# peterbudai/redux

Hardware: AMD Instinct MI355X
Metric: encode MB/s (whole node), per-block bitstream bit-exact (higher is better)
Workload: dtype u32

## Files before the change

redux_amd/csrc/redux_encode.hpp:

```cpp
#pragma once

#include "redux_coder.hpp"

#include "../../include/redux_hip.h"

#include <hip/hip_runtime.h>
#include <stdint.h>

namespace redux {

__global__ void k_fill_rc(double *rc, uint32_t n)
{
    const uint32_t i = blockIdx.x * blockDim.x + threadIdx.x;
    if (i < n) {
        const double r = 1.0 / (double)(257u + i);
        rc[i] = __longlong_as_double(__double_as_longlong(r) + 4);
    }
}

struct EncCore {
    const uint8_t *in;
    uint64_t       in_len;
    uint64_t       nblocks;
    uint8_t       *slots;
    uint64_t       slot_bytes;
    uint32_t      *sizes;
    int32_t       *status;
};

struct EncArgs : EncCore {
    const double  *rc;
    uint32_t       block_size;
    uint32_t       slot_cap;
    uint32_t       nfreeze;
    uint32_t       code_bits;
    uint32_t       aligned16;
    uint32_t       lanes;
    uint32_t      *claims;
    const redux_block *table;
    uint32_t       pair_width;
    uint32_t       win0, winlen;
    double         rc_frozen;
    uint32_t      *cstate, *cbase;
};
static_assert(sizeof(EncCore) == 56 && sizeof(EncArgs) == 144, "kernarg layout");

constexpr uint32_t kIdleEntry = 0xFFFFFFFFu;

struct EncLane {
    uint32_t soff, len;
    uint64_t ob;
};
__device__ __forceinline__ EncLane enc_lane(const EncArgs &a, uint64_t blk0, uint64_t blk, uint32_t lane, bool live, const uint8_t *&wsrc)
{
    EncLane L;
    if (a.table) {
        const redux_block e = a.table[live ? blk : blk0];
        wsrc   = a.in;
        L.soff = (uint32_t)e.offset;
        L.len  = live ? e.length : 0u;
        L.ob   = e.index;
    } else {
        wsrc   = a.in + blk0 * a.block_size;
        L.soff = live ? lane * a.block_size : 0u;
        L.len  = 0;
        if (live) {
            const uint64_t rem = a.in_len - blk * a.block_size;
            L.len              = rem < a.block_size ? (uint32_t)rem : a.block_size;
        }
        L.ob = blk;
    }
    return L;
}

__device__ __forceinline__ uint32_t wave_min(uint32_t v)
{
#pragma unroll
    for (int o = 32; o > 0; o >>= 1) {
        const uint32_t w = __shfl_xor(v, o);
        v = w < v ? w : v;
    }
    return v;
}
__device__ __forceinline__ uint32_t wave_max(uint32_t v)
{
#pragma unroll
    for (int o = 32; o > 0; o >>= 1) {
        const uint32_t w = __shfl_xor(v, o);
        v = w > v ? w : v;
    }
    return v;
}

template <bool U16, bool FIXUP, bool UPD>
__device__ __forceinline__ void encode_chunk(const Tree<U16> &T, EncState &S, const uint4 cur, uint32_t p,
                                             uint32_t nfreeze, rc_ptr rc, uint32_t sh, uint8_t *wdst)
{
    const uint32_t w[4] = {cur.x, cur.y, cur.z, cur.w};
    double         r[16];
#pragma unroll
    for (int i = 0; i < 16; i++)
        r[i] = rc[UPD ? p + i : nfreeze];
#pragma unroll
    for (int i = 0; i < 16; i++) {
        const uint32_t s   = (w[i >> 2] >> (8 * (i & 3))) & 0xFFu;
        const uint32_t nup = UPD ? p + i : nfreeze;
        uint32_t       lo, hi;
        T.template get_frequency<UPD>(s, nup, true, lo, hi);
        encode_symbol_fast<FIXUP>(S, lo, hi, 257u + nup, r[i], sh, wdst);
    }
}

template <bool U16, bool FIXUP>
__global__ void __launch_bounds__(64) k_encode(EncArgs a)
{
    __shared__ uint32_t lds[Tree<U16>::kDwords];
    const uint32_t lane = threadIdx.x;
    const uint64_t blk0 = (uint64_t)blockIdx.x * a.lanes;
    const uint64_t blk  = blk0 + lane;
    const bool     live = lane < a.lanes && blk < a.nblocks && !(a.table && a.table[blk].index == kIdleEntry);

    for (uint32_t i = lane; i < Tree<U16>::kDwords / 4; i += 64)
        reinterpret_cast<uint4 *>(lds)[i] = make_uint4(0, 0, 0, 0);
    __syncthreads();
    Tree<U16> T;
    T.init(lds, lane);

    const uint8_t *wsrc;
    const EncLane  EL    = enc_lane(a, blk0, blk, lane, live, wsrc);
    const uint32_t len   = EL.len, soff = EL.soff;
    uint8_t       *wdst  = a.slots + blk0 * a.slot_bytes;
    const uint32_t off0  = live ? lane * (uint32_t)a.slot_bytes
                                : (a.lanes == 1 ? 0u : (uint32_t)(a.nblocks - blk0) * (uint32_t)a.slot_bytes);
    const uint32_t limit = off0 + a.slot_cap;

    const uint32_t minlen  = __builtin_amdgcn_readfirstlane(wave_min(live ? len : 0xFFFFFFFFu));
    constexpr uint32_t kChunkBudget = 16 * 4 + 32;
    const uint32_t maxlen  = __builtin_amdgcn_readfirstlane(wave_max(live ? len : 0u));
    const uint32_t sh      = 32 - a.code_bits;
    const uint32_t nfreeze = a.nfreeze;
    const rc_ptr   rc      = (rc_ptr)a.rc;

    EncState S;
    enc_init(S, off0);

    uint32_t p        = 0;
    uint32_t main_end = 0;
    if (a.aligned16 && minlen != 0xFFFFFFFFu && minlen > 16)
        main_end = (minlen - 1) & ~15u;

    if (main_end) {
        const uint32_t a_end = main_end < (nfreeze & ~15u) ? main_end : (nfreeze & ~15u);
        if (p < a_end) {
            uint4 cur = *reinterpret_cast<const uint4 *>(wsrc + soff);
            for (; p < a_end; p += 16) {
                if (__builtin_amdgcn_ballot_w64(S.off + kChunkBudget > limit)) {
                    main_end = p;
                    break;
                }
                uint4 nxt = cur;
                if (p + 16 < a_end)
                    nxt = *reinterpret_cast<const uint4 *>(wsrc + soff + p + 16);
                encode_chunk<U16, FIXUP, true>(T, S, cur, p, nfreeze, rc, sh, wdst);
                cur = nxt;
            }
        }
        if (p < main_end && p < nfreeze) {
            const uint32_t m_end = p + 16;
            for (; p < m_end; p++) {
                const uint32_t nup = p < nfreeze ? p : nfreeze;
                uint32_t       lo, hi;
                T.template get_frequency<true>(wsrc[soff + p], nup, p < nfreeze, lo, hi);
                encode_symbol<FIXUP>(S, lo, hi, 257u + nup, rc[nup], sh, false, wdst, limit);
            }
        }
        if (p < main_end) {
            uint4 cur = *reinterpret_cast<const uint4 *>(wsrc + soff + p);
            for (; p < main_end; p += 16) {
                if (__builtin_amdgcn_ballot_w64(S.off + kChunkBudget > limit)) {
                    main_end = p;
                    break;
                }
                uint4 nxt = cur;
                if (p + 16 < main_end)
                    nxt = *reinterpret_cast<const uint4 *>(wsrc + soff + p + 16);
                encode_chunk<U16, FIXUP, false>(T, S, cur, p, nfreeze, rc, sh, wdst);
                cur = nxt;
            }
        }
    }

    for (; p <= maxlen; p++) {
        const uint32_t nup = p < nfreeze ? p : nfreeze;
        const double   r   = rc[nup];
        const uint32_t c   = 257u + nup;
        if (live && p < len) {
            uint32_t lo, hi;
            T.template get_frequency<true>(wsrc[soff + p], nup, p < nfreeze && p + 1 != len, lo, hi);
            encode_symbol<FIXUP>(S, lo, hi, c, r, sh, false, wdst, limit);
        } else if (live && p == len) {
            const uint32_t shifts = encode_symbol<FIXUP>(S, c - 1, c, c, r, sh, true, wdst, limit);
            const uint32_t size   = encode_finish(S, shifts, a.code_bits, off0, wdst, limit);
            a.sizes[EL.ob]  = size;
            a.status[EL.ob] = size > a.slot_cap ? REDUX_OUTPUT_TOO_SMALL : REDUX_OK;
        }
    }
}

constexpr uint32_t kRingSlots = 8;
constexpr uint32_t kRingBytes = 2 * kRingSlots * 64 * 8;

__device__ __forceinline__ void pair_barrier()
{
    asm volatile("s_waitcnt lgkmcnt(0)\n\ts_barrier" ::: "memory");
}

struct ChunkQueue {
    const uint8_t *base;
    uint32_t       soff;
    uint32_t       last;
    uint32_t       nextp;
    uint32_t       idx;
    uint4          c[8], n[8];

    __device__ __forceinline__ void prefetch()
    {
#pragma unroll
        for (int i = 0; i < 8; i++) {
            const uint32_t p = nextp + 16 * i;
            n[i] = *reinterpret_cast<const uint4 *>(base + soff + (p < last ? p : last));
        }
        nextp += 128;
    }
    __device__ __forceinline__ void swap()
    {
#pragma unroll
        for (int i = 0; i < 8; i++)
            c[i] = n[i];
        idx = 0;
        prefetch();
    }
    __device__ __forceinline__ void init(const uint8_t *b, uint32_t so, uint32_t e)
    {
        base = b; soff = so; last = e - 16; nextp = 0;
        prefetch();
        swap();
    }
    __device__ __forceinline__ uint4 pop()
    {
        uint4 r;
        switch (idx) {
        case 0: r = c[0]; break;
        case 1: r = c[1]; break;
        case 2: r = c[2]; break;
        case 3: r = c[3]; break;
        case 4: r = c[4]; break;
        case 5: r = c[5]; break;
        case 6: r = c[6]; break;
        default: r = c[7]; break;
        }
        if (++idx == 8)
            swap();
        return r;
    }
};

constexpr int kPairStride = 256 | kSwapped;
__device__ __forceinline__ uint32_t ring_at(uint32_t i, uint32_t lane)
{
    return (i >> 1) * 128u + lane * 2u + (i & 1u);
}
constexpr int kMaskAhead = 8;
static_assert(kMaskAhead == 4 || kMaskAhead == 8, "prime() covers these");
static_assert(16 % kMaskAhead == 0, "slot i % AHEAD must mean the same in every chunk");
struct MaskPipe {
    uint4    s[kMaskAhead], m[kMaskAhead];
    uint32_t four;
    __amdgpu_buffer_rsrc_t rsrc;
    __device__ __forceinline__ void init()
    {
        rsrc = __builtin_amdgcn_make_buffer_rsrc(const_cast<uint32_t *>(k_mask_table.v), 0, sizeof k_mask_table.v, 0x00027000);
        four = 4;
        asm volatile("" : "+v"(four));
    }
    __device__ __forceinline__ uint32_t row_of(int K, uint32_t w) const
    {
        uint32_t off;
        if (K == 0)
            asm("v_lshlrev_b32_sdwa %0, %1, %2 dst_sel:DWORD dst_unused:UNUSED_PAD src0_sel:DWORD src1_sel:BYTE_0" : "=v"(off) : "v"(four), "v"(w));
        else if (K == 1)
            asm("v_lshlrev_b32_sdwa %0, %1, %2 dst_sel:DWORD dst_unused:UNUSED_PAD src0_sel:DWORD src1_sel:BYTE_1" : "=v"(off) : "v"(four), "v"(w));
        else if (K == 2)
            asm("v_lshlrev_b32_sdwa %0, %1, %2 dst_sel:DWORD dst_unused:UNUSED_PAD src0_sel:DWORD src1_sel:BYTE_2" : "=v"(off) : "v"(four), "v"(w));
        else
            asm("v_lshlrev_b32_sdwa %0, %1, %2 dst_sel:DWORD dst_unused:UNUSED_PAD src0_sel:DWORD src1_sel:BYTE_3" : "=v"(off) : "v"(four), "v"(w));
        return off;
    }
    __device__ __forceinline__ void load(int slot, uint32_t row)
    {
        const char *e = reinterpret_cast<const char *>(k_mask_table.v) + row;
        (void)e;
        const auto r0 = __builtin_amdgcn_raw_buffer_load_b128(rsrc, row, 0, 0), r1 = __builtin_amdgcn_raw_buffer_load_b128(rsrc, row + 16u, 0, 0);
        s[slot] = make_uint4(r0[0], r0[1], r0[2], r0[3]);
        m[slot] = make_uint4(r1[0], r1[1], r1[2], r1[3]);
        const uint32_t sym = row >> 4;
    }
    __device__ __forceinline__ void prime(const uint4 cur)
    {
        init();
        const uint32_t w[2] = {cur.x, cur.y};
        load(0, row_of(0, w[0])); load(1, row_of(1, w[0])); load(2, row_of(2, w[0])); load(3, row_of(3, w[0]));
        if (kMaskAhead == 8) {
            load(4 % kMaskAhead, row_of(0, w[1])); load(5 % kMaskAhead, row_of(1, w[1]));
            load(6 % kMaskAhead, row_of(2, w[1])); load(7 % kMaskAhead, row_of(3, w[1]));
        }
    }
};

template <bool UPD>
__device__ __forceinline__ void model_chunk(const Tree<true> &T, uint2 *ring, uint32_t lane, const uint4 cur, const uint4 nxt,
                                            MaskPipe &mp, uint32_t p, uint32_t nfreeze, uint32_t *top = nullptr)
{
    constexpr int kInFlight = UPD ? 7 : 8;
    const uint32_t w[8] = {cur.x, cur.y, cur.z, cur.w, nxt.x, nxt.y, nxt.z, nxt.w};
    auto sym = [&](int i) { return (w[i >> 2] >> (8 * (i & 3))) & 0xFFu; };
    constexpr int D = 1;
    Tree<true>::Nodes q[D + 1];
    uint2             held = make_uint2(0, 0);
    constexpr bool kMasked = UPD && D == 1;
#pragma unroll
    for (int d = 0; d < D; d++)
        q[d] = kMasked ? T.issue_masked(sym(d), mp.s[d % kMaskAhead], top) : T.template issue<UPD>(sym(d), true, top);
#pragma unroll
    for (int i = 0; i < 16; i++) {
        const uint32_t s   = sym(i);
        const uint32_t nup = UPD ? p + i : nfreeze;
        const bool late = i == 7;
        if (i + D < 16 && !late) {
            q[D] = kMasked ? T.issue_masked(sym(i + D), mp.s[(i + D) % kMaskAhead], top) : T.template issue<UPD>(sym(i + D), true, top);
            __builtin_amdgcn_sched_barrier(0);
        }
        uint32_t lo, hi;
        if (D == 1 && i + D < 16 && !late && i != 8 && i != 0 && kInFlight == 7)
        {
            if (i & 1)
                __builtin_amdgcn_s_waitcnt(0xC00F | 0x70 | (7 << 8));
            else
                __builtin_amdgcn_s_waitcnt(0xC00F | 0x70 | (8 << 8));
        }
        T.finish_tab(s, nup, q[0], mp.s[i % kMaskAhead], mp.m[i % kMaskAhead], lo, hi);
        mp.load(i % kMaskAhead, mp.row_of((i + kMaskAhead) & 3, w[(i + kMaskAhead) >> 2]));
        if (i & 1) {
            *reinterpret_cast<uint4 *>(ring + ring_at(i - 1, lane)) = make_uint4(held.x, held.y, lo, hi);
        } else
            held = make_uint2(lo, hi);
        if (late) {
            __builtin_amdgcn_sched_barrier(0);
            q[D] = kMasked ? T.issue_masked(sym(i + D), mp.s[(i + D) % kMaskAhead], top) : T.template issue<UPD>(sym(i + D), true, top);
            if (kInFlight == 7)
                asm volatile("s_waitcnt lgkmcnt(7)\n\ts_barrier" ::: "memory");
            else
                asm volatile("s_waitcnt lgkmcnt(8)\n\ts_barrier" ::: "memory");
        } else if ((i & 7) == 7)
            pair_barrier();
#pragma unroll
        for (int d = 0; d < D; d++)
            q[d] = q[d + 1];
    }
}

template <bool FIXUP, int MODE, bool CB32>
__device__ __forceinline__ void coder_chunk(EncState &S, const uint2 *ring, uint32_t lane, uint32_t p,
                                            uint32_t nfreeze, rc_ptr rc, uint32_t sh, uint8_t *wdst, double (&r)[8])
{
#pragma unroll
    for (int h = 0; h < 2; h++) {
        pair_barrier();
        uint2 lh[8];
#pragma unroll
        for (int i = 0; i < 8; i += 2) {
            const uint4 two = *reinterpret_cast<const uint4 *>(ring + ring_at(h * 8 + i, lane));
            lh[i]     = make_uint2(two.x, two.y);
            lh[i + 1] = make_uint2(two.z, two.w);
        }
        double rn[8];
        if (MODE == 0) {
            uint32_t zero;
            asm volatile("s_mov_b32 %0, 0" : "=s"(zero) : "v"(lh[0].x));
            const rc_ptr nb = rc + (p + 8u * h + 8u + zero);
#pragma unroll
            for (int i = 0; i < 8; i++)
                rn[i] = nb[i];
        }
        const EncState S0  = S;
        SpecCarry      C   = spec_begin(S);
        uint32_t       mx  = 0;
#pragma unroll
        for (int i = 0; i < 8; i++) {
            const uint32_t nup = MODE == 0 ? p + h * 8 + i : nfreeze;
            asm volatile("" : "+v"(lh[i].y));
            const uint32_t hi = lh[i].y;
            const uint32_t m = encode_symbol_spec<FIXUP, CB32, kPairStride>(S, C, lh[i].x, hi, 257u + nup, MODE == 0 ? r[i] : rc[nfreeze], sh, wdst);
            mx               = m > mx ? m : mx;
        }
        spec_end(S, C);
        const uint64_t bad = __builtin_amdgcn_ballot_w64(mx > 32u);
        if (__builtin_expect(bad != 0, 0)) {
            S = S0;
#pragma unroll
            for (int i = 0; i < 8; i++) {
                const uint32_t nup = MODE == 0 ? p + h * 8 + i : nfreeze;
                encode_symbol<FIXUP, kPairStride>(S, lh[i].x, lh[i].y, 257u + nup, MODE == 0 ? r[i] : rc[nfreeze], sh, false, wdst, 0xFFFFFFFFu);
            }
        }
        if (MODE == 0) {
#pragma unroll
            for (int i = 0; i < 8; i++)
                r[i] = rn[i];
        }
    }
}

template <bool FIXUP>
__device__ __forceinline__ void coder_chunk_checked(EncState &S, const uint2 *ring, uint32_t lane, uint32_t p,
                                                    uint32_t nfreeze, rc_ptr rc, uint32_t sh, uint8_t *wdst,
                                                    uint32_t limit)
{
    for (uint32_t i = 0; i < 16; i++) {
        if ((i & 7) == 0)
            pair_barrier();
        const uint2    lh  = ring[ring_at(i, lane)];
        const uint32_t q   = p + i;
        const uint32_t nup = q < nfreeze ? q : nfreeze;
        encode_symbol<FIXUP, kPairStride>(S, lh.x, lh.y, 257u + nup, rc[nup], sh, false, wdst, limit);
    }
}

constexpr uint32_t kClaimWords = 2048;
constexpr uint32_t kPairDwords = Tree<true>::kDwords + kRingBytes / 4;

template <bool FIXUP, bool CB32>
__global__ void __launch_bounds__(128) k_encode_pair(EncArgs a)
{
    __shared__ uint32_t lds[kPairDwords];
    const uint32_t w8   = __builtin_amdgcn_readfirstlane(threadIdx.x >> 6);
    const uint32_t lane = threadIdx.x & 63;
    const uint64_t blk0 = (uint64_t)blockIdx.x * a.lanes;
    const uint64_t blk  = blk0 + lane;
    const bool     live = lane < a.lanes && blk < a.nblocks && !(a.table && a.table[blk].index == kIdleEntry);

    for (uint32_t i = threadIdx.x; i < Tree<true>::kDwords / 4; i += 128)
        reinterpret_cast<uint4 *>(lds)[i] = make_uint4(0, 0, 0, 0);
    uint32_t role = w8;
    uint2   *ring = reinterpret_cast<uint2 *>(lds + Tree<true>::kDwords);
    uint32_t claim_delta = 0;
    {
        uint32_t hwid, xcc;
        asm volatile("s_getreg_b32 %0, hwreg(HW_REG_HW_ID)" : "=s"(hwid));
        asm volatile("s_getreg_b32 %0, hwreg(HW_REG_XCC_ID)" : "=s"(xcc));
        volatile uint32_t *book = reinterpret_cast<volatile uint32_t *>(ring) + kRingBytes / 4 - 4;
        if (lane == 0)
            book[w8] = (hwid >> 4) & 3u;
        __syncthreads();
        uint32_t *claim_word = a.claims + (((xcc & 7u) << 8) | ((hwid >> 8) & 0xFFu));
        if (w8 == 0 && lane == 0) {
            const uint32_t s0 = book[0], s1 = book[1];
            const uint32_t straight = (1u << (4 * s0)) | (1u << (16 + 4 * s1));
            const uint32_t flipped  = (1u << (4 * s1)) | (1u << (16 + 4 * s0));
            uint32_t       old      = __hip_atomic_load(claim_word, __ATOMIC_RELAXED, __HIP_MEMORY_SCOPE_AGENT);
            uint32_t       flip;
            do {
                const uint32_t cs = ((old >> (4 * s0)) & 15u) + ((old >> (16 + 4 * s1)) & 15u);
                const uint32_t cf = ((old >> (4 * s1)) & 15u) + ((old >> (16 + 4 * s0)) & 15u);
                flip              = cf < cs;
            } while (!__hip_atomic_compare_exchange_strong(claim_word, &old, old + (flip ? flipped : straight),
                                                           __ATOMIC_RELAXED, __ATOMIC_RELAXED, __HIP_MEMORY_SCOPE_AGENT));
            book[2] = flip;
            book[3] = flip ? flipped : straight;
        }
        __syncthreads();
        role ^= __builtin_amdgcn_readfirstlane(book[2]);
        claim_delta = book[3];
    }
    const uint32_t wave = role;
    Tree<true> T;
    T.init(lds, lane);

    const uint8_t *wsrc;
    const EncLane  EL    = enc_lane(a, blk0, blk, lane, live, wsrc);
    const uint32_t len   = EL.len, soff = EL.soff;
    uint8_t       *wdst  = a.slots + (uint64_t)blockIdx.x * (64 * a.slot_bytes + 128);
    const uint32_t off0  = lane * 4u;
    const uint32_t limit = off0 + (a.slot_cap / 4u) * 256u;

    const uint32_t minlen  = __builtin_amdgcn_readfirstlane(wave_min(live ? len : 0xFFFFFFFFu));
    const uint32_t maxlen  = __builtin_amdgcn_readfirstlane(wave_max(live ? len : 0u));
    const uint32_t sh      = 32 - a.code_bits;
    const uint32_t nfreeze = a.nfreeze;
    const rc_ptr   rc      = (rc_ptr)a.rc;
    constexpr uint32_t kChunkBudget = (16 * 4 + 32) * (stride_of<kPairStride> / 4);

    uint32_t main_end = 0;
    if (a.aligned16 && minlen != 0xFFFFFFFFu && minlen > 16)
        main_end = (minlen - 1) & ~15u;
    const uint32_t a_end = main_end < (nfreeze & ~15u) ? main_end : (nfreeze & ~15u);
    const uint32_t m_end = (a_end < main_end && a_end < nfreeze) ? a_end + 16 : a_end;

    EncState S;
    enc_init(S, off0);

    if (wave == 0) {
        __builtin_amdgcn_s_setprio(3);
        if (main_end) {
            uint32_t p = 0;
            ChunkQueue Q;
            Q.init(wsrc, soff, main_end);
#define NEXT_CHUNK() Q.pop()
            uint4    cur = NEXT_CHUNK(), nxt;
            MaskPipe mp;
            mp.prime(cur);
            uint32_t top = 0;
            for (; p < a_end; p += 16, cur = nxt) {
                nxt = NEXT_CHUNK();
                model_chunk<true>(T, ring, lane, cur, nxt, mp, p, nfreeze, &top);
            }
            T.add(T.A[7], top);
            for (; p < m_end; p += 16) {
                for (uint32_t i = 0; i < 16; i++) {
                    const uint32_t q   = p + i;
                    const uint32_t nup = q < nfreeze ? q : nfreeze;
                    uint32_t       lo, hi;
                    T.template get_frequency<true>(wsrc[soff + q], nup, q < nfreeze, lo, hi);
                    ring[ring_at(i, lane)] = make_uint2(lo, hi);
                    if ((i & 7) == 7)
                        pair_barrier();
                }
                cur = NEXT_CHUNK();
                mp.prime(cur);
            }
            for (; p < main_end; p += 16, cur = nxt) {
                nxt = NEXT_CHUNK();
                model_chunk<false>(T, ring, lane, cur, nxt, mp, p, nfreeze);
            }
#undef NEXT_CHUNK
        }
    } else {
        uint32_t p = 0;
        double   r[8];
        uint32_t r_at = ~0u;
        for (; p < main_end; p += 16) {
            if (__builtin_amdgcn_ballot_w64(S.off + kChunkBudget > limit) || (p >= a_end && p < m_end))
                coder_chunk_checked<FIXUP>(S, ring, lane, p, nfreeze, rc, sh, wdst, limit);
            else if (p < a_end) {
                if (r_at != p) {
#pragma unroll
                    for (int i = 0; i < 8; i++)
                        r[i] = rc[p + i];
                }
                coder_chunk<FIXUP, 0, CB32>(S, ring, lane, p, nfreeze, rc, sh, wdst, r);
                r_at = p + 16;
            } else
                coder_chunk<FIXUP, 1, CB32>(S, ring, lane, p, nfreeze, rc, sh, wdst, r);
        }
    }
    __syncthreads();
    if (wave == 0)
        return;

    for (uint32_t p = main_end; p <= maxlen; p++) {
        const uint32_t nup = p < nfreeze ? p : nfreeze;
        const double   r   = rc[nup];
        const uint32_t c   = 257u + nup;
        if (live && p < len) {
            uint32_t lo, hi;
            T.template get_frequency<true>(wsrc[soff + p], nup, p < nfreeze && p + 1 != len, lo, hi);
            encode_symbol<FIXUP, kPairStride>(S, lo, hi, c, r, sh, false, wdst, limit);
        } else if (live && p == len) {
            const uint32_t shifts = encode_symbol<FIXUP, kPairStride>(S, c - 1, c, c, r, sh, true, wdst, limit);
            const uint32_t size   = encode_finish<kPairStride>(S, shifts, a.code_bits, off0, wdst, limit);
            a.sizes[EL.ob]  = size;
            a.status[EL.ob] = size > a.slot_cap ? REDUX_OUTPUT_TOO_SMALL : REDUX_OK;
        }
    }
    if (lane == 0) {
        uint32_t hwid, xcc;
        asm volatile("s_getreg_b32 %0, hwreg(HW_REG_HW_ID)" : "=s"(hwid));
        asm volatile("s_getreg_b32 %0, hwreg(HW_REG_XCC_ID)" : "=s"(xcc));
        __hip_atomic_fetch_sub(a.claims + (((xcc & 7u) << 8) | ((hwid >> 8) & 0xFFu)), claim_delta, __ATOMIC_RELAXED,
                               __HIP_MEMORY_SCOPE_AGENT);
    }
}

}
```

Measured before the change: 369,700.

## Move input chunk prefetch from model wave to coder wave via LDS feed slot

The global-memory input prefetch queue moves from the modelling wave (wave 0) to the coder wave. The coder wave now pops each 16-byte chunk and writes it into a ring slot in LDS that the model wave has already consumed, and the model wave reads its next chunk from that slot instead of holding an 8-deep register queue. This takes global-load latency and register pressure off the critical model wave. The cost is extra LDS traffic and a tighter dependence on the barrier ordering between the two waves. A pinned variant of the queue adds an explicit waitcnt and register pinning so the compiler cannot sink the loads.

```diff
diff --git a/redux_amd/csrc/redux_encode.hpp b/redux_amd/csrc/redux_encode.hpp
--- a/redux_amd/csrc/redux_encode.hpp
+++ b/redux_amd/csrc/redux_encode.hpp
@@ -215,7 +215,8 @@
     asm volatile("s_waitcnt lgkmcnt(0)\n\ts_barrier" ::: "memory");
 }
 
-struct ChunkQueue {
+template <bool PIN>
+struct ChunkQueueT {
     const uint8_t *base;
     uint32_t       soff;
     uint32_t       last;
@@ -234,17 +235,30 @@
     }
     __device__ __forceinline__ void swap()
     {
+        if (PIN)
+            __builtin_amdgcn_s_waitcnt(0x0F70);
 #pragma unroll
         for (int i = 0; i < 8; i++)
             c[i] = n[i];
+        if (PIN) {
+            typedef uint32_t u32x4 __attribute__((ext_vector_type(4)));
+#pragma unroll
+            for (int i = 0; i < 8; i++) {
+                u32x4 t = {c[i].x, c[i].y, c[i].z, c[i].w};
+                asm volatile("" : "+v"(t));
+                c[i] = make_uint4(t[0], t[1], t[2], t[3]);
+            }
+            __builtin_amdgcn_sched_barrier(0);
+        }
         idx = 0;
         prefetch();
     }
-    __device__ __forceinline__ void init(const uint8_t *b, uint32_t so, uint32_t e)
+    __device__ __forceinline__ void init(const uint8_t *b, uint32_t so, uint32_t e, uint32_t first = 0)
     {
         base = b; soff = so; last = e - 16; nextp = 0;
         prefetch();
         swap();
+        idx = first;
     }
     __device__ __forceinline__ uint4 pop()
     {
@@ -264,11 +278,16 @@
         return r;
     }
 };
+using ChunkQueue = ChunkQueueT<false>;
 
 constexpr int kPairStride = 256 | kSwapped;
 __device__ __forceinline__ uint32_t ring_at(uint32_t i, uint32_t lane)
 {
     return (i >> 1) * 128u + lane * 2u + (i & 1u);
+}
+__device__ __forceinline__ uint4 *feed_slot(uint2 *ring, uint32_t lane)
+{
+    return reinterpret_cast<uint4 *>(ring + ring_at(0, lane));
 }
 constexpr int kMaskAhead = 8;
 static_assert(kMaskAhead == 4 || kMaskAhead == 8, "prime() covers these");
@@ -370,7 +389,7 @@
 }
 
 template <bool FIXUP, int MODE, bool CB32>
-__device__ __forceinline__ void coder_chunk(EncState &S, const uint2 *ring, uint32_t lane, uint32_t p,
+__device__ __forceinline__ void coder_chunk(EncState &S, uint2 *ring, uint32_t lane, uint32_t p, const uint4 feed,
                                             uint32_t nfreeze, rc_ptr rc, uint32_t sh, uint8_t *wdst, double (&r)[8])
 {
 #pragma unroll
@@ -383,6 +402,8 @@
             lh[i]     = make_uint2(two.x, two.y);
             lh[i + 1] = make_uint2(two.z, two.w);
         }
+        if (h == 0)
+            *feed_slot(ring, lane) = feed;
         double rn[8];
         if (MODE == 0) {
             uint32_t zero;
@@ -422,13 +443,15 @@
 }
 
 template <bool FIXUP>
-__device__ __forceinline__ void coder_chunk_checked(EncState &S, const uint2 *ring, uint32_t lane, uint32_t p,
+__device__ __forceinline__ void coder_chunk_checked(EncState &S, uint2 *ring, uint32_t lane, uint32_t p, const uint4 feed,
                                                     uint32_t nfreeze, rc_ptr rc, uint32_t sh, uint8_t *wdst,
                                                     uint32_t limit)
 {
     for (uint32_t i = 0; i < 16; i++) {
         if ((i & 7) == 0)
             pair_barrier();
+        if (i == 2)
+            *feed_slot(ring, lane) = feed;
         const uint2    lh  = ring[ring_at(i, lane)];
         const uint32_t q   = p + i;
         const uint32_t nup = q < nfreeze ? q : nfreeze;
@@ -513,10 +536,9 @@
         __builtin_amdgcn_s_setprio(3);
         if (main_end) {
             uint32_t p = 0;
-            ChunkQueue Q;
-            Q.init(wsrc, soff, main_end);
-#define NEXT_CHUNK() Q.pop()
-            uint4    cur = NEXT_CHUNK(), nxt;
+            *feed_slot(ring, lane) = *reinterpret_cast<const uint4 *>(wsrc + soff + (main_end > 16 ? 16u : 0u));
+#define NEXT_CHUNK() (*feed_slot(ring, lane))
+            uint4    cur = *reinterpret_cast<const uint4 *>(wsrc + soff), nxt;
             MaskPipe mp;
             mp.prime(cur);
             uint32_t top = 0;
@@ -526,6 +548,7 @@
             }
             T.add(T.A[7], top);
             for (; p < m_end; p += 16) {
+                nxt = NEXT_CHUNK();
                 for (uint32_t i = 0; i < 16; i++) {
                     const uint32_t q   = p + i;
                     const uint32_t nup = q < nfreeze ? q : nfreeze;
@@ -535,7 +558,7 @@
                     if ((i & 7) == 7)
                         pair_barrier();
                 }
-                cur = NEXT_CHUNK();
+                cur = nxt;
                 mp.prime(cur);
             }
             for (; p < main_end; p += 16, cur = nxt) {
@@ -548,19 +571,23 @@
         uint32_t p = 0;
         double   r[8];
         uint32_t r_at = ~0u;
+        ChunkQueueT<true> Q;
+        if (main_end)
+            Q.init(wsrc, soff, main_end, 2);
         for (; p < main_end; p += 16) {
+            const uint4 feed = Q.pop();
             if (__builtin_amdgcn_ballot_w64(S.off + kChunkBudget > limit) || (p >= a_end && p < m_end))
-                coder_chunk_checked<FIXUP>(S, ring, lane, p, nfreeze, rc, sh, wdst, limit);
+                coder_chunk_checked<FIXUP>(S, ring, lane, p, feed, nfreeze, rc, sh, wdst, limit);
             else if (p < a_end) {
                 if (r_at != p) {
 #pragma unroll
                     for (int i = 0; i < 8; i++)
                         r[i] = rc[p + i];
                 }
-                coder_chunk<FIXUP, 0, CB32>(S, ring, lane, p, nfreeze, rc, sh, wdst, r);
+                coder_chunk<FIXUP, 0, CB32>(S, ring, lane, p, feed, nfreeze, rc, sh, wdst, r);
                 r_at = p + 16;
             } else
-                coder_chunk<FIXUP, 1, CB32>(S, ring, lane, p, nfreeze, rc, sh, wdst, r);
+                coder_chunk<FIXUP, 1, CB32>(S, ring, lane, p, feed, nfreeze, rc, sh, wdst, r);
         }
     }
     __syncthreads();
```

After: 381,600, median of 6. +3.2%, better.
